# facebookresearch/SlowFast

Measured on AMD Instinct MI355X. Metric: clips/sec (fwd+bwd), SlowFast-8x8-R50 32x224^2 synthetic clips, per-GPU batch 32, higher is better.
Workload: dtype fp16; 1 GPU; SLOWFAST_8x8_R50: forward + cross_entropy loss + backward + sgd step, inputs resident in HBM, per-GPU batch 32; global_batch=32, parallelism=dp1, launch=hip-graph(fwd+bwd) + eager all-reduce/optimizer, optimizer=FlatOptimizer (fused unscale+norm+clip+update, dynamic loss scale on device)

## Files before the change

include/sfamd.h:

```cpp
#ifndef SFAMD_H
#define SFAMD_H
#include <stddef.h>
#include <stdint.h>
#ifdef __cplusplus
extern "C" {
#endif

#define SF_ABI_VERSION 32
typedef void* sf_stream_t;

typedef struct sf_conv_desc {
    int32_t N, Ci, Ti, Hi, Wi;
    int32_t Co, To, Ho, Wo;
    int32_t kT, kH, kW;
    int32_t sT, sH, sW;
    int32_t pT, pH, pW;
    int32_t dT, dH, dW;
    int32_t Cw;
    int32_t ldx, ldy;
    int32_t Cow;
} sf_conv_desc;

int sf_abi_version(void);
const char* sf_backend(void);
// ... 51 lines not shown
                     int32_t ldy, const float* scale, const float* shift, int relu_self, float* part,
                     sf_stream_t stream);
int sf_bn_bwd_finalize(float* part, int32_t nblk, int32_t C, int32_t Creal, float count, const float* gamma, const float* mean,
                       const float* rstd, float inv_loss_scale, float* dgamma, float* dbeta, int accumulate,
                       float* coef, sf_stream_t stream);
int sf_bn_bwd_apply(int64_t M, int32_t C, const void* dz, int32_t lddz, const void* zmask, int32_t ldm, const void* y,
                    int32_t ldy, const float* scale, const float* shift, int relu_self, const float* coef, void* dy,
                    int32_t lddy, void* gout, int32_t ldg, sf_stream_t stream);

int sf_pool_fwd(int32_t N, int32_t T, int32_t H, int32_t W, int32_t C, int32_t kH, int32_t kW, int32_t sH, int32_t sW,
                int32_t pH, int32_t pW, const void* y, int32_t ldy, const float* scale, const float* shift, int relu,
                void* out, int32_t ldo, void* argmax, int32_t cls, sf_stream_t stream);
int sf_pool_bwd(int32_t N, int32_t T, int32_t H, int32_t W, int32_t C, int32_t kH, int32_t kW, int32_t sH, int32_t sW,
                int32_t pH, int32_t pW, const void* pooled, int32_t ldp, const void* argmax, int relu,
                const void* dout, int32_t lddo, void* g, int32_t ldg, int32_t cls, sf_stream_t stream);

int sf_pool3d_fwd(int32_t N, int32_t T, int32_t H, int32_t W, int32_t C, int32_t kT, int32_t kH, int32_t kW, const void* x,
                  int32_t ldx, void* out, int32_t ldo, void* argmax, sf_stream_t stream);
int sf_pool3d_bwd(int32_t N, int32_t T, int32_t H, int32_t W, int32_t C, int32_t kT, int32_t kH, int32_t kW,
                  const void* argmax, const void* dout, int32_t lddo, void* dx, int32_t lddx, sf_stream_t stream);

int sf_ncthw_to_cl(const float* x, int32_t N, int32_t C, int64_t S, int32_t Cp, void* out, sf_stream_t stream);
int sf_cl_to_ncthw(const void* x, int32_t ld, int32_t N, int32_t C, int64_t S, float* out, sf_stream_t stream);


int sf_bgemm(int64_t M, int32_t N, int32_t K, const void* A, int32_t lda, const void* W, int32_t ldw, const float* bias,
             const void* resid, int32_t ldr, void* Y, int32_t ldy, int32_t nbatch, int32_t bh, int64_t sa_b, int64_t sa_h,
             int64_t sw_b, int64_t sw_h, int64_t sy_b, int64_t sy_h, int64_t sr_b, int64_t sr_h, int32_t resid_row0,
             float alpha, sf_stream_t stream);
typedef struct sf_rows32 {
// ... 222 lines not shown
```

slowfast_amd/csrc/sf_api.hip:

```cpp
#include "../../include/sfamd.h"
#include "sf_bn.h"
#include "sf_common.h"
#include "sf_igemm.h"
#include "sf_igemm2.h"
#include "sf_wgrad2.h"
#include "sf_cbwd.h"
#include "sf_pool.h"
#include "sf_dwconv.h"
#include "sf_dwsweep.h"
#include "sf_dwtemporal.h"
#include "sf_tokens.h"
#include "sf_x3d.h"
#include "sf_stem.h"
#include "sf_attn.h"
#include "sf_roi.h"
#include "sf_optim.h"
#include "sf_mixup.h"
#include "sf_erase.h"
#include "sf_pack.h"
#include "sf_sample.h"
#include "sf_color.h"
#include "sf_randaug.h"
#include "sf_hog.h"
#include "sf_pixel.h"
// ... 1122 lines not shown

extern "C" int sf_pool_bwd(int32_t N, int32_t T, int32_t H, int32_t W, int32_t C, int32_t kH, int32_t kW, int32_t sH,
                           int32_t sW, int32_t pH, int32_t pW, const void* pooled, int32_t ldp, const void* argmax,
                           int relu, const void* dout, int32_t lddo, void* g, int32_t ldg, int32_t cls,
                           sf_stream_t stream) {
    PoolParams p;
    if (fill_pool(p, N, T, H, W, C, kH, kW, sH, sW, pH, pW, nullptr, 0, nullptr, nullptr, relu)) return -1;
    REQUIRE(argmax && dout && g, "sf_pool_bwd: null pointer");
    (void)pooled; (void)ldp;
    p.cls = cls ? 1 : 0; p.fdT = make_fastdiv(T);
    p.out = (f16*)g; p.ldo = ldg; p.dout = (const f16*)dout; p.lddo = lddo;
    p.pooled = (const f16*)pooled; p.ldp = ldp; p.argmax = (uint8_t*)argmax;
    p.fdW = make_fastdiv(W); p.fdH = make_fastdiv(H);
    p.total = (int64_t)N * T * H * W * (C / 8);
    REQUIRE(p.total < (1ll << 31), "sf_pool_bwd: too many elements");
    p.fdsH = make_fastdiv(sH); p.fdsW = make_fastdiv(sW);
    if (kH <= 2 * sH && kW <= 2 * sW)
        hipLaunchKernelGGL(sf_pool_bwd4_kernel, dim3(pool_grid(p.total + (int64_t)N * (C / 8))), dim3(SF_THREADS), 0,
                           (hipStream_t)stream, p);
    else
        hipLaunchKernelGGL(sf_pool_bwd_kernel, dim3(pool_grid(p.total + (int64_t)N * (C / 8))), dim3(SF_THREADS), 0,
                           (hipStream_t)stream, p);
    return check_launch("pool_bwd");
}

extern "C" int sf_pool3d_fwd(int32_t N, int32_t T, int32_t H, int32_t W, int32_t C, int32_t kT, int32_t kH, int32_t kW,
                             const void* x, int32_t ldx, void* out, int32_t ldo, void* argmax, sf_stream_t stream) {
    REQUIRE(x && out && argmax && C > 0 && C % 8 == 0 && kT > 0 && kH > 0 && kW > 0 && kT * kH * kW <= 255,
            "sf_pool3d_fwd: bad arguments");
    Pool3dParams p;
    p.N = N; p.T = T; p.H = H; p.W = W; p.C = C; p.kT = kT; p.kH = kH; p.kW = kW;
    p.To = T / kT; p.Ho = H / kH; p.Wo = W / kW;
    REQUIRE(p.To > 0 && p.Ho > 0 && p.Wo > 0, "sf_pool3d_fwd: window larger than the input");
    p.x = (const f16*)x; p.ldx = ldx; p.out = (f16*)out; p.ldo = ldo; p.argmax = (uint8_t*)argmax;
    p.dout = nullptr; p.lddo = 0;
    p.fdG = make_fastdiv(C / 8); p.fdW = make_fastdiv(p.Wo); p.fdH = make_fastdiv(p.Ho); p.fdT = make_fastdiv(p.To);
    p.total = (int64_t)N * p.To * p.Ho * p.Wo * (C / 8);
    REQUIRE(p.total < (1ll << 31), "sf_pool3d_fwd: too many elements");
// ... 2079 lines not shown
```

slowfast_amd/csrc/sf_bn.h:

```cpp
#pragma once
#include "sf_common.h"

struct RowTile {
    int M, C;
    int rows_per_block;
    __device__ __forceinline__ bool init(int& gcol, int& r0, int& r1, int& rstep, int bx = (int)blockIdx.x) const {
        const int G = C >> 3;
        const int TG = G < SF_THREADS ? G : SF_THREADS;
        const int rpi = SF_THREADS / TG;
        const int tx = threadIdx.x % TG, ty = threadIdx.x / TG;
        gcol = blockIdx.y * SF_THREADS + tx;
        r0 = bx * rows_per_block + ty;
        r1 = (bx + 1) * rows_per_block;
        if (r1 > M) r1 = M;
        rstep = rpi;
        return ty < rpi && gcol < G;
    }
};

__device__ __forceinline__ void load8f(const float* p, float (&v)[8]) {
#pragma unroll
    for (int e = 0; e < 8; ++e) v[e] = p[e];
}

// ... 227 lines not shown
    for (int e = 0; e < 8; ++e) g[e] = (float)dz[e];
    if (bits_ptr) {
        const uint32_t b = *bits_ptr;
#pragma unroll
        for (int e = 0; e < 8; ++e) g[e] = ((b >> e) & 1u) ? g[e] : 0.f;
    } else if (zmask_ptr) {
        f16x8 z = ld16(zmask_ptr);
#pragma unroll
        for (int e = 0; e < 8; ++e) g[e] = ((float)z[e] > 0.f) ? g[e] : 0.f;
    } else if (relu_self) {
#pragma unroll
        for (int e = 0; e < 8; ++e) g[e] = ((float)yv[e] * sc[e] + sh[e] > 0.f) ? g[e] : 0.f;
    }
}

__global__ __launch_bounds__(SF_THREADS) void sf_bn_bwd_reduce_kernel(BnBwdReduceParams p) {
    __shared__ float s_red[SF_THREADS][17];
    int gcol, r0, r1, rstep;
    const bool active = p.rt.init(gcol, r0, r1, rstep);
    const int c = gcol * 8;
    float sg[8], sgy[8], sc[8], sh[8];
#pragma unroll
    for (int e = 0; e < 8; ++e) { sg[e] = 0.f; sgy[e] = 0.f; sc[e] = 1.f; sh[e] = 0.f; }
    if (active) {
        if (p.relu_self) { load8f(p.scale + c, sc); load8f(p.shift + c, sh); }
        for (int m = r0; m < r1; m += rstep) {
            f16x8 dz = ld16(p.dz + (int64_t)m * p.lddz + c);
            f16x8 yv = ld16(p.y + (int64_t)m * p.ldy + c);
            float g[8];
            const bool bitm = p.zmask && p.ldm == 0;
            masked_grad8(dz, yv, (p.zmask && !bitm) ? p.zmask + (int64_t)m * p.ldm + c : nullptr, p.relu_self, sc, sh, g,
                         bitm ? reinterpret_cast<const uint8_t*>(p.zmask) + (int64_t)m * (p.rt.C >> 3) + gcol : nullptr);
#pragma unroll
            for (int e = 0; e < 8; ++e) { sg[e] += g[e]; sgy[e] += g[e] * (float)yv[e]; }
        }
    }
    rowtile_reduce_store(p.rt, active, c, sg, sgy, p.part + (int64_t)blockIdx.x * 2 * p.rt.C, s_red);
}

struct BnBwdFinalizeParams {
    const float* part; int nblk; int row_stride; int C; int Creal;
    float count;
    const float* gamma; const float* mean; const float* rstd;
    float inv_loss_scale;
    float* dgamma; float* dbeta;
    int accumulate;
    float* coef;
};

__global__ __launch_bounds__(SF_FIN_THREADS_MAX) void sf_bn_bwd_finalize_kernel(BnBwdFinalizeParams p) {
    __shared__ double s_s[SF_FIN_SEG_MAX][SF_FIN_CH];
    __shared__ double s_q[SF_FIN_SEG_MAX][SF_FIN_CH];
// ... 25 lines not shown

struct BnBwdApplyParams {
    RowTile rt;
    const f16* dz; int lddz;
    const f16* zmask; int ldm;
    const f16* y; int ldy;
    const float* scale; const float* shift;
    int relu_self;
    const float* coef;
    f16* dy; int lddy;
    f16* gout; int ldg;
    const float* sample_add;
    FastDiv fdS;
};

__global__ __launch_bounds__(SF_THREADS) void sf_bn_bwd_apply_kernel(BnBwdApplyParams p) {
    int gcol, r0, r1, rstep;
    if (!p.rt.init(gcol, r0, r1, rstep)) return;
    const int c = gcol * 8, C = p.rt.C;
    float sc[8], sh[8], k1[8], k2[8], k3[8];
#pragma unroll
    for (int e = 0; e < 8; ++e) { sc[e] = 1.f; sh[e] = 0.f; }
    if (p.relu_self) { load8f(p.scale + c, sc); load8f(p.shift + c, sh); }
    load8f(p.coef + c, k1);
    load8f(p.coef + C + c, k2);
    load8f(p.coef + 2 * C + c, k3);
    for (int m = r0; m < r1; m += rstep) {
        f16x8 dz = ld16(p.dz + (int64_t)m * p.lddz + c);
        f16x8 yv = ld16(p.y + (int64_t)m * p.ldy + c);
        float g[8];
        const bool bitm = p.zmask && p.ldm == 0;
        masked_grad8(dz, yv, (p.zmask && !bitm) ? p.zmask + (int64_t)m * p.ldm + c : nullptr, p.relu_self, sc, sh, g,
                     bitm ? reinterpret_cast<const uint8_t*>(p.zmask) + (int64_t)m * (C >> 3) + gcol : nullptr);
        f16x8 o;
        if (p.sample_add) {
            float ad[8];
            load8f(p.sample_add + (int64_t)fd_div((uint32_t)m, p.fdS) * C + c, ad);
#pragma unroll
            for (int e = 0; e < 8; ++e) g[e] += ad[e];
        }
#pragma unroll
        for (int e = 0; e < 8; ++e) o[e] = (f16)(k1[e] * g[e] + k2[e] + k3[e] * (float)yv[e]);
        st16(p.dy + (int64_t)m * p.lddy + c, o);
        if (p.gout) {
            f16x8 go;
#pragma unroll
            for (int e = 0; e < 8; ++e) go[e] = (f16)g[e];
            st16(p.gout + (int64_t)m * p.ldg + c, go);
        }
    }
}
```

slowfast_amd/csrc/sf_pool.h:

```cpp
#pragma once
#include "sf_common.h"

struct PoolParams {
    const f16* y; int ldy;
    const float* scale; const float* shift; int relu;
    int N, T, H, W, C;
    int Ho, Wo;
    int kH, kW, sH, sW, pH, pW;
    f16* out; int ldo;
    uint8_t* argmax;
    const f16* pooled; int ldp;
    const f16* dout; int lddo;
    FastDiv fdG, fdW, fdH;
    int64_t total;
    int cls;
    FastDiv fdT;
    FastDiv fdsH, fdsW;
};

__device__ __forceinline__ int64_t pool_row(const PoolParams& p, uint32_t nt, int Hx, int Wx, int h, int w) {
    int64_t r = ((int64_t)nt * Hx + h) * Wx + w;
    if (p.cls) r += fd_div(nt, p.fdT) + 1;
    return r;
}
// ... 108 lines not shown
                const f16x8 d = ld16(p.dout + orow * p.lddo + c);
#pragma unroll
                for (int e = 0; e < 8; ++e) {
                    const uint32_t a = ((e < 4 ? pk.x : pk.y) >> (8 * (e & 3))) & 0xffu;
                    g[e] += a == me ? (float)d[e] : 0.f;
                }
            }
        }
        f16x8 o;
#pragma unroll
        for (int e = 0; e < 8; ++e) o[e] = (f16)g[e];
        st16(p.out + pool_row(p, nt, p.H, p.W, (int)h, (int)w) * p.ldo + c, o);
    }
}

__global__ __launch_bounds__(SF_THREADS) void sf_pool_bwd4_kernel(PoolParams p) {
    const int64_t ncls = p.cls ? (int64_t)p.N * (p.C >> 3) : 0;
    for (int64_t idx = (int64_t)blockIdx.x * SF_THREADS + threadIdx.x; idx < p.total + ncls;
         idx += (int64_t)gridDim.x * SF_THREADS) {
        if (idx >= p.total) {
            const int64_t j = idx - p.total;
            const int G = p.C >> 3;
            const int64_t n = j / G;
            const int c = (int)(j % G) * 8;
            st16(p.out + n * ((int64_t)p.T * p.H * p.W + 1) * p.ldo + c,
                 ld16(p.dout + n * ((int64_t)p.T * p.Ho * p.Wo + 1) * p.lddo + c));
            continue;
        }
        uint32_t q, gcol, w, h, nt;
        fd_divmod((uint32_t)idx, p.fdG, q, gcol);
        fd_divmod(q, p.fdW, q, w);
        fd_divmod(q, p.fdH, nt, h);
        const int c = gcol * 8;
        const int hh = (int)fd_div(h + (uint32_t)p.pH, p.fdsH), wh = (int)fd_div(w + (uint32_t)p.pW, p.fdsW);
        int hoc[2], woc[2], khs[2], kws[2];
        bool hv[2], wv[2];
#pragma unroll
        for (int a = 0; a < 2; ++a) {
            const int ho = hh - 1 + a, wo = wh - 1 + a;
            khs[a] = (int)h - (ho * p.sH - p.pH);
            kws[a] = (int)w - (wo * p.sW - p.pW);
            hv[a] = ho >= 0 && ho < p.Ho && khs[a] < p.kH;
            wv[a] = wo >= 0 && wo < p.Wo && kws[a] < p.kW;
            hoc[a] = ho < 0 ? 0 : (ho > p.Ho - 1 ? p.Ho - 1 : ho);
            woc[a] = wo < 0 ? 0 : (wo > p.Wo - 1 ? p.Wo - 1 : wo);
        }
        u32x2 pk[2][2];
        f16x8 d[2][2];
#pragma unroll
        for (int a = 0; a < 2; ++a)
#pragma unroll
            for (int b = 0; b < 2; ++b) {
                const int64_t orow = pool_row(p, nt, p.Ho, p.Wo, hoc[a], woc[b]);
                pk[a][b] = *reinterpret_cast<const u32x2*>(p.argmax + orow * p.C + c);
                d[a][b] = ld16(p.dout + orow * p.lddo + c);
            }
        float g[8];
#pragma unroll
        for (int e = 0; e < 8; ++e) g[e] = 0.f;
#pragma unroll
        for (int a = 0; a < 2; ++a)
#pragma unroll
            for (int b = 0; b < 2; ++b) {
                const bool on = hv[a] && wv[b];
                const uint32_t me = (uint32_t)(khs[a] * p.kW + kws[b]);
#pragma unroll
                for (int e = 0; e < 8; ++e) {
                    const uint32_t am = ((e < 4 ? pk[a][b].x : pk[a][b].y) >> (8 * (e & 3))) & 0xffu;
                    g[e] += on && am == me ? (float)d[a][b][e] : 0.f;
                }
            }
        f16x8 o;
#pragma unroll
        for (int e = 0; e < 8; ++e) o[e] = (f16)g[e];
        st16(p.out + pool_row(p, nt, p.H, p.W, (int)h, (int)w) * p.ldo + c, o);
    }
}

struct Pool3dParams {
    int N, T, H, W, C, kT, kH, kW, To, Ho, Wo;
    const f16* x; int ldx;
    f16* out; int ldo;
    uint8_t* argmax;
    const f16* dout; int lddo;
    FastDiv fdG, fdW, fdH, fdT;
    int64_t total;
};
__global__ __launch_bounds__(SF_THREADS) void sf_pool3d_fwd_kernel(Pool3dParams p) {
    for (int64_t idx = (int64_t)blockIdx.x * SF_THREADS + threadIdx.x; idx < p.total;
         idx += (int64_t)gridDim.x * SF_THREADS) {
        uint32_t q, gcol, wo, ho, to, n;
// ... 239 lines not shown
```

slowfast_amd/engine.py:

```python
import functools
import os

import torch

from . import lib as _sflib

from . import ops

_f16 = _sflib.act_dtype()
_listeners = []
FORCE_WEIGHT_PREP = False
PARAM_EPOCH = 0
PACK_RECORD = None
PACK_PLAN = os.environ.get("SF_PACK_PLAN", "1") != "0"
BN_FUSE_REDUCE = os.environ.get("SF_BN_FUSE_REDUCE", "1") != "0"
CAT_IN_PLACE = os.environ.get("SF_CAT_IN_PLACE", "1") != "0"
SEGMENTS = None


class _Segments:
    def __init__(self):
        self.cuts = []

    def cut(self, tensors):
# ... 373 lines not shown
        return geom if ops.conv_c_bwd_plan(geom) is not None else None

    def fused_c_backward(self, geom, x, dz, y, st, bits, part=None, bn_fuse=None):
        bn = self.bn
        dgamma, dbeta, accumulate = self._bn_grad_dest()
        coef = ops.bn_bwd_coef(dz, y, bn.weight, st.mean, st.rstd, dgamma, dbeta, zmask=bits, inv_loss_scale=1.0,
                               accumulate=accumulate, part=part)
        dw, zero_first = _grad_dest(self.conv.weight)
        _, wd = self.weights(geom)
        fuse = None
        if bn_fuse is not None:
            y0, st0 = bn_fuse
            fuse = (y0, st0.scale, st0.shift)
        return ops.conv_c_bwd(dz, bits, y, coef, x, wd, geom, dw, bn=fuse, out_scale=1.0, zero_first=zero_first)

    def bn_backward(self, dz, y, st, zmask=None, relu_self=False, want_g=False, part=None):
        bn = self.bn
        dgamma, dbeta, accumulate = self._bn_grad_dest()
        return ops.bn_bwd(dz, y, bn.weight, st.mean, st.rstd, dgamma, dbeta, zmask=zmask,
                          relu_affine=(st.scale, st.shift) if relu_self else None, inv_loss_scale=1.0,
                          accumulate=accumulate, want_g=want_g, sync=_sync_of(bn), part=part)

    def params(self):
        p = [self.conv.weight]
        if self.conv.bias is not None:
            p.append(self.conv.bias)
        if self.bn is not None:
            p += [self.bn.weight, self.bn.bias]
        return p

    def _fold_source(self, w):
        return w

    def fold(self):
        w = self.conv.weight.detach().float()
        b = self.conv.bias.detach().float() if self.conv.bias is not None else None
# ... 107 lines not shown
        assert k[0] == 1 and s[0] == 1 and p[0] == 0, "stem pooling is spatial-only in every reference config"
        out, arg = ops.pool_fwd(y, k[1:], s[1:], p[1:], affine=(st.scale, st.shift, True))
        if CAPTURE is not None:
            CAPTURE.append({"kind": "stem", "mod": mod, "raw": [y], "bn": [(st.scale, st.shift)], "out": out,
                            "argmax": torch.where(arg == 255, torch.zeros_like(arg), arg)})
        ctx.mod, ctx.xcl, ctx.y, ctx.st = mod, xcl, y, st
        ctx.pool = (tuple(k[1:]), tuple(s[1:]), tuple(p[1:]))
        ctx.pooled, ctx.arg = out, arg
        return out

    @staticmethod
    @delivers_grads
    def backward(ctx, dout):
        unit = ctx.mod._unit
        st = ctx.st
        g = ops.pool_bwd(ctx.y.shape, ctx.pooled, ctx.arg, as_cl(dout), *ctx.pool, relu=True)
        dy = unit.bn_backward(g, ctx.y, st)
        unit.backward(ctx.xcl, None, dy, need_dx=False)
        _notify(unit.params())
        ctx.xcl = ctx.y = ctx.pooled = ctx.arg = None
        return (None, None) + param_grads(ctx, 2)


class FuseFn(torch.autograd.Function):

    @staticmethod
    def forward(ctx, x_s, x_f, mod, *params):
        record_params(ctx, params)
        unit = mod._unit
        x_s, x_f = as_cl(x_s), as_cl(x_f)
        yf, st = unit.forward(x_f, None, mod.training)
        N, Cs, T, H, W = x_s.shape
# ... 165 lines not shown
```

slowfast_amd/lib.py:

```python
import ctypes
import os
from ctypes import POINTER, Structure, c_char_p, c_float, c_int, c_int32, c_int64, c_void_p

_HERE = os.path.dirname(os.path.abspath(__file__))
ABI_VERSION = 32
ACT_MODE = os.environ.get("SF_ACT_DTYPE", "fp16").lower()
if ACT_MODE not in ("fp16", "bf16"):
    raise ValueError(f"SF_ACT_DTYPE={ACT_MODE!r}: expected fp16 or bf16")
DEFAULT_LIBRARY = os.path.join(_HERE, "libsfamd.so" if ACT_MODE == "fp16" else "libsfamd_bf16.so")


def act_dtype():
    import torch
    return torch.float16 if ACT_MODE == "fp16" else torch.bfloat16


def act_eps():
    return 2.0 ** -11 if ACT_MODE == "fp16" else 2.0 ** -8


class ConvDesc(Structure):

    _fields_ = [(n, c_int32) for n in (
        "N", "Ci", "Ti", "Hi", "Wi", "Co", "To", "Ho", "Wo", "kT", "kH", "kW", "sT", "sH", "sW",
# ... 61 lines not shown
    "sf_bn_bwd_blocks": (c_int, [c_int64, c_int32]),
    "sf_flat_blocks": (c_int, [c_int64]),
    "sf_flat_sumsq": (c_int, [_F, c_int64, _F, _P]),
    "sf_step_control": (c_int, [_F, c_int32, _F, c_float, c_float, c_int, c_float, c_float, c_int32, _P]),
    "sf_flat_sgd": (c_int, [_F, _F, _F, _P, _P, _P, c_int32, _F, _P, _P, c_int32, c_float, c_float, c_float, c_int, _P]),
    "sf_flat_adamw": (c_int, [_F, _F, _F, _F, _P, _P, _P, c_int32, _F, _P, _P, c_int32, c_float, c_float, c_float, c_float, _P]),
    "sf_flat_sgd_tab": (c_int, [_F, _F, _F, _P, _P, _P, c_int32, _F, _F, _F, c_float, c_float, c_float, c_int, _P]),
    "sf_flat_adamw_tab": (c_int, [_F, _F, _F, _F, _P, _P, _P, c_int32, _F, _F, _F, c_float, c_float, c_float, c_float, _P]),
    "sf_flat_lars_trust": (c_int, [_F, _F, _P, _P, _P, c_int32, _P, c_int32, _F, _F, _P, _F, c_float, c_float, c_float, _P]),
    "sf_bn_bwd_reduce": (c_int, [c_int64, c_int32, _P, c_int32, _P, c_int32, _P, c_int32, _F, _F, c_int, _F, _P]),
    "sf_bn_bwd_finalize": (c_int, [_F, c_int32, c_int32, c_int32, c_float, _F, _F, _F, c_float, _F, _F, c_int, _F, _P]),
    "sf_bn_bwd_apply": (c_int, [c_int64, c_int32, _P, c_int32, _P, c_int32, _P, c_int32, _F, _F, c_int, _F, _P,
                                c_int32, _P, c_int32, _P]),
    "sf_pool_fwd": (c_int, [c_int32] * 11 + [_P, c_int32, _F, _F, c_int, _P, c_int32, _P, c_int32, _P]),
    "sf_pool_bwd": (c_int, [c_int32] * 11 + [_P, c_int32, _P, c_int, _P, c_int32, _P, c_int32, c_int32, _P]),
    "sf_pool3d_fwd": (c_int, [c_int32] * 8 + [_P, c_int32, _P, c_int32, _P, _P]),
    "sf_pool3d_bwd": (c_int, [c_int32] * 8 + [_P, _P, c_int32, _P, c_int32, _P]),
    "sf_ncthw_to_cl": (c_int, [_F, c_int32, c_int32, c_int64, c_int32, _P, _P]),
    "sf_cl_to_ncthw": (c_int, [_P, c_int32, c_int32, c_int32, c_int64, _F, _P]),
    "sf_bgemm": (c_int, [c_int64, c_int32, c_int32, _P, c_int32, _P, c_int32, _F, _P, c_int32, _P, c_int32, c_int32,
                         c_int32] + [c_int64] * 8 + [c_int32, c_float, _P]),
    "sf_bgemm_tn": (c_int, [c_int64, c_int32, c_int32, _P, c_int32, _P, c_int32, _P, c_int32, c_float, c_int32, c_int32]
                    + [c_int64] * 6 + [_P]),
    "sf_layernorm_fwd": (c_int, [c_int64, c_int32, _P, c_int32, _F, _F, c_float, _P, c_int32, _F, _F, _P]),
    "sf_gemm_rows32": (c_int, [c_int64, c_int32, c_int32, _P, c_int32, _P, c_int32, _F, _P, c_int32, _P, c_int32,
                               POINTER(Rows32), _P]),
    "sf_layernorm_fwd_rows32": (c_int, [c_int64, c_int32, _P, c_int32, _F, _F, c_float, _P, c_int32, _F, _F,
                                        POINTER(Rows32), _P]),
    "sf_layernorm_bwd_blocks": (c_int, [c_int64, c_int32]),
    "sf_layernorm_bwd": (c_int, [c_int64, c_int32, _P, c_int32, _P, c_int32, _F, _F, _F, _P, c_int32, _P, c_int32, _F, _P]),
# ... 160 lines not shown
```

slowfast_amd/ops.py:

```python
from ctypes import byref, c_int32, c_int64

import torch

from . import lib as _sflib

from .lib import ConvDesc, SfError, get_lib

_f16 = _sflib.act_dtype()


def _triple(v):
    return tuple(v) if isinstance(v, (tuple, list)) else (v, v, v)


def _stream(t):
    if t.is_cuda:
        return torch.cuda.current_stream(t.device).cuda_stream
    if get_lib().backend != "hostsim":
        raise SfError("slowfast_amd kernels need CUDA/HIP tensors (got a CPU tensor and the gfx950 library)")
    return None


def _ptr(t):
    return None if t is None else t.data_ptr()
# ... 283 lines not shown

def bn_act(y, scale=None, shift=None, relu=False, resid=None, rscale=None, rshift=None, out=None, want_mask=False):
    ldy = cl_ld(y)
    N, C, T, H, W = y.shape
    out = cl_empty(y.shape, y.device) if out is None else out
    assert tuple(out.shape) == tuple(y.shape)
    mask = torch.empty((rows(y), C // 8), dtype=torch.uint8, device=y.device) if want_mask else None
    get_lib().call("sf_bn_act", rows(y), C, y.data_ptr(), ldy, _ptr(scale), _ptr(shift), _ptr(resid),
                   cl_ld(resid) if resid is not None else 0, _ptr(rscale), _ptr(rshift), int(bool(relu)),
                   out.data_ptr(), cl_ld(out), _ptr(mask), _stream(y),
                   work=dict(bytes=2.0 * y.numel() * (2 + int(resid is not None) + (1 / 16 if want_mask else 0))))
    return (out, mask) if want_mask else out


def bn_bwd(dz, y, gamma, mean, rstd, dgamma, dbeta, zmask=None, relu_affine=None, inv_loss_scale=1.0,
           accumulate=False, want_g=False, out=None, sync=None, part=None, sample_add=None, coef_only=False):
    lib = get_lib()
    N, C, T, H, W = y.shape
    M = rows(y)
    s = _stream(y)
    fused_part = part
    if fused_part is None:
        nblk = lib.call("sf_bn_bwd_blocks", M, C)
        part = torch.empty((nblk, 2, C), dtype=torch.float32, device=y.device)
    else:
        assert part.dtype == torch.float32 and part.is_contiguous() and tuple(part.shape[1:]) == (2, C)
        nblk = part.shape[0]
    sc, sh = (relu_affine if relu_affine is not None else (None, None))
    relu_self = int(relu_affine is not None)
    bits = zmask is not None and zmask.dtype == torch.uint8
    if bits:
        assert zmask.numel() == M * (C // 8) and zmask.is_contiguous()
    mcost = 0.0 if zmask is None else (1 / 16 if bits else 1.0)
    lddz, ldy, ldm = cl_ld(dz), cl_ld(y), (0 if bits or zmask is None else cl_ld(zmask))
    if fused_part is None:
        lib.call("sf_bn_bwd_reduce", M, C, dz.data_ptr(), lddz, _ptr(zmask), ldm, y.data_ptr(), ldy, _ptr(sc), _ptr(sh),
                 relu_self, part.data_ptr(), s, work=dict(bytes=2.0 * y.numel() * (2 + mcost)))
    coef = torch.empty((3, C), dtype=torch.float32, device=y.device)
    if sync is None:
        lib.call("sf_bn_bwd_finalize", part.data_ptr(), nblk, C, gamma.numel(), float(M), gamma.data_ptr(), mean.data_ptr(),
                 rstd.data_ptr(), float(inv_loss_scale), dgamma.data_ptr(), dbeta.data_ptr(), int(accumulate),
                 coef.data_ptr(), s)
    else:
        import torch.distributed as dist
        group, gsize = sync
        tot = part.sum(0, keepdim=True)
        loc = tot.clone()
        lib.call("sf_bn_bwd_finalize", loc.data_ptr(), 1, C, gamma.numel(), float(M), gamma.data_ptr(), mean.data_ptr(),
                 rstd.data_ptr(), float(inv_loss_scale), dgamma.data_ptr(), dbeta.data_ptr(), int(accumulate),
                 coef.data_ptr(), s)
        dist.all_reduce(tot, group=group)
        scratch = torch.empty((2, gamma.numel()), dtype=torch.float32, device=y.device)
        lib.call("sf_bn_bwd_finalize", tot.data_ptr(), 1, C, gamma.numel(), float(M) * gsize, gamma.data_ptr(),
                 mean.data_ptr(), rstd.data_ptr(), float(inv_loss_scale), scratch[0].data_ptr(), scratch[1].data_ptr(), 0,
                 coef.data_ptr(), s)
    if coef_only:
        return coef
    dy = cl_empty(y.shape, y.device) if out is None else out
    if sample_add is not None:
        assert fused_part is not None and zmask is None and relu_affine is None and not want_g
        assert sample_add.dtype == torch.float32 and sample_add.is_contiguous() and tuple(sample_add.shape) == (N, C)
        lib.call("sf_bn_bwd_apply_sample", M, C, dz.data_ptr(), lddz, y.data_ptr(), ldy, coef.data_ptr(), sample_add.data_ptr(),
                 M // N, dy.data_ptr(), cl_ld(dy), s, work=dict(bytes=2.0 * y.numel() * 3))
        return dy
    g = cl_empty(y.shape, y.device) if want_g else None
    lib.call("sf_bn_bwd_apply", M, C, dz.data_ptr(), lddz, _ptr(zmask), ldm, y.data_ptr(), ldy, _ptr(sc), _ptr(sh),
             relu_self, coef.data_ptr(), dy.data_ptr(), cl_ld(dy), _ptr(g), cl_ld(g) if g is not None else 0, s,
             work=dict(bytes=2.0 * y.numel() * (3 + mcost + int(want_g))))
    return (dy, g) if want_g else dy


def bn_bwd_coef(dz, y, gamma, mean, rstd, dgamma, dbeta, zmask=None, inv_loss_scale=1.0, accumulate=False, part=None):
    return bn_bwd(dz, y, gamma, mean, rstd, dgamma, dbeta, zmask=zmask, inv_loss_scale=inv_loss_scale, accumulate=accumulate,
                  part=part, coef_only=True)


def conv_c_bwd_plan(geom, in_affine=False, mask_bits=True):
    tile_rows, ws = c_int32(0), c_int64(0)
    ok = get_lib().call("sf_conv_c_bwd_plan", byref(geom.desc(geom.Ci, geom.Co)), int(bool(in_affine)), int(bool(mask_bits)),
                        byref(tile_rows), byref(ws))
    return (tile_rows.value, ws.value) if ok == 1 else None


def conv_c_bwd(dz, bits, yc, coef, act, wd, geom, dw, bn=None, out_scale=1.0, zero_first=True, out=None):
    plan = conv_c_bwd_plan(geom)
    assert plan is not None, "conv_c_bwd: the planner rejects this geometry"
    tile_rows, ws_bytes = plan
    assert tuple(act.shape) == geom.in_shape and tuple(dz.shape) == geom.out_shape and tuple(yc.shape) == geom.out_shape
    assert dw.dtype == torch.float32 and dw.is_contiguous() and dw.numel() == geom.Cow * geom.Cw * geom.taps
# ... 50 lines not shown
```

Before: 904.2 clips/s.

## Fuse stem max-pool backward gather into BN backward reduce and apply kernels

The stem pool's backward no longer materializes the unpooled gradient tensor. The BN backward reduce and apply kernels now recompute the 2x2 argmax gather from the pooled gradient on the fly, so one full-resolution write and two reads of the stem activation gradient are avoided. The gather is done twice (once in reduce, once in apply), which adds index arithmetic and repeated small reads of argmax and dout. A test hook can switch the new path off, and the original path remains as a fallback.

```diff
diff --git a/include/sfamd.h b/include/sfamd.h
--- a/include/sfamd.h
+++ b/include/sfamd.h
@@ -6,7 +6,7 @@
 extern "C" {
 #endif
 
-#define SF_ABI_VERSION 32
+#define SF_ABI_VERSION 33
 typedef void* sf_stream_t;
 
 typedef struct sf_conv_desc {
@@ -89,6 +89,15 @@
 int sf_pool_bwd(int32_t N, int32_t T, int32_t H, int32_t W, int32_t C, int32_t kH, int32_t kW, int32_t sH, int32_t sW,
                 int32_t pH, int32_t pW, const void* pooled, int32_t ldp, const void* argmax, int relu,
                 const void* dout, int32_t lddo, void* g, int32_t ldg, int32_t cls, sf_stream_t stream);
+
+int sf_bn_bwd_pool_plan(int32_t C, int32_t kH, int32_t kW, int32_t sH, int32_t sW, int32_t cls);
+int sf_bn_bwd_reduce_pool(int32_t N, int32_t T, int32_t H, int32_t W, int32_t C, int32_t kH, int32_t kW, int32_t sH, int32_t sW,
+                          int32_t pH, int32_t pW, const void* argmax, const void* dout, int32_t lddo, const void* y, int32_t ldy,
+                          const float* scale, const float* shift, int relu_self, float* part, sf_stream_t stream);
+int sf_bn_bwd_apply_pool(int32_t N, int32_t T, int32_t H, int32_t W, int32_t C, int32_t kH, int32_t kW, int32_t sH, int32_t sW,
+                         int32_t pH, int32_t pW, const void* argmax, const void* dout, int32_t lddo, const void* y, int32_t ldy,
+                         const float* scale, const float* shift, int relu_self, const float* coef, void* dy, int32_t lddy,
+                         sf_stream_t stream);
 
 int sf_pool3d_fwd(int32_t N, int32_t T, int32_t H, int32_t W, int32_t C, int32_t kT, int32_t kH, int32_t kW, const void* x,
                   int32_t ldx, void* out, int32_t ldo, void* argmax, sf_stream_t stream);
diff --git a/slowfast_amd/csrc/sf_api.hip b/slowfast_amd/csrc/sf_api.hip
--- a/slowfast_amd/csrc/sf_api.hip
+++ b/slowfast_amd/csrc/sf_api.hip
@@ -1160,6 +1160,7 @@
     p.fdW = make_fastdiv(W); p.fdH = make_fastdiv(H);
     p.total = (int64_t)N * T * H * W * (C / 8);
     REQUIRE(p.total < (1ll << 31), "sf_pool_bwd: too many elements");
+    REQUIRE((int64_t)N * T * p.Ho * p.Wo + N < (1ll << 31), "sf_pool_bwd: too many pooled positions");
     p.fdsH = make_fastdiv(sH); p.fdsW = make_fastdiv(sW);
     if (kH <= 2 * sH && kW <= 2 * sW)
         hipLaunchKernelGGL(sf_pool_bwd4_kernel, dim3(pool_grid(p.total + (int64_t)N * (C / 8))), dim3(SF_THREADS), 0,
@@ -1168,6 +1169,70 @@
         hipLaunchKernelGGL(sf_pool_bwd_kernel, dim3(pool_grid(p.total + (int64_t)N * (C / 8))), dim3(SF_THREADS), 0,
                            (hipStream_t)stream, p);
     return check_launch("pool_bwd");
+}
+
+extern "C" int sf_bn_bwd_pool_plan(int32_t C, int32_t kH, int32_t kW, int32_t sH, int32_t sW, int32_t cls) {
+    if (test_hook("SF_STEM_POOL_FUSE", 1) == 0) return 0;
+    return C > 0 && C % 8 == 0 && kH > 0 && kW > 0 && sH > 0 && sW > 0 && kH <= 2 * sH && kW <= 2 * sW && !cls ? 1 : 0;
+}
+static int fill_pool_grad(const char* who, PoolParams& q, int32_t N, int32_t T, int32_t H, int32_t W, int32_t C, int32_t kH,
+                          int32_t kW, int32_t sH, int32_t sW, int32_t pH, int32_t pW, const void* argmax, const void* dout,
+                          int32_t lddo, int64_t& M) {
+    REQUIRE(sf_bn_bwd_pool_plan(C, kH, kW, sH, sW, 0) == 1,
+            "%s: this pool keeps sf_pool_bwd + sf_bn_bwd_reduce + sf_bn_bwd_apply (sf_bn_bwd_pool_plan == 0)", who);
+    REQUIRE(N > 0 && T > 0 && H > 0 && W > 0 && pH >= 0 && pW >= 0 && pH < kH && pW < kW && H + 2 * pH >= kH && W + 2 * pW >= kW,
+            "%s: bad pool geometry", who);
+    if (fill_pool(q, N, T, H, W, C, kH, kW, sH, sW, pH, pW, nullptr, 0, nullptr, nullptr, 1)) return -1;
+    REQUIRE(argmax && dout && lddo >= C, "%s: null pointer or short pitch", who);
+    M = (int64_t)N * T * H * W;
+    if (check_rows(who, M, C)) return -1;
+    REQUIRE((int64_t)N * T * q.Ho * q.Wo < (1ll << 31), "%s: too many pooled positions", who);
+    q.cls = 0; q.fdT = make_fastdiv(T);
+    q.dout = (const f16*)dout; q.lddo = lddo; q.argmax = (uint8_t*)argmax;
+    q.fdW = make_fastdiv(W); q.fdH = make_fastdiv(H);
+    q.fdsH = make_fastdiv(sH); q.fdsW = make_fastdiv(sW);
+    q.total = M * (C / 8);
+    return 0;
+}
+
+extern "C" int sf_bn_bwd_reduce_pool(int32_t N, int32_t T, int32_t H, int32_t W, int32_t C, int32_t kH, int32_t kW, int32_t sH,
+                                     int32_t sW, int32_t pH, int32_t pW, const void* argmax, const void* dout, int32_t lddo,
+                                     const void* y, int32_t ldy, const float* scale, const float* shift, int relu_self,
+                                     float* part, sf_stream_t stream) {
+    PoolParams q;
+    int64_t M;
+    if (fill_pool_grad("sf_bn_bwd_reduce_pool", q, N, T, H, W, C, kH, kW, sH, sW, pH, pW, argmax, dout, lddo, M)) return -1;
+    REQUIRE(y && part && ldy >= C, "sf_bn_bwd_reduce_pool: null pointer or short pitch");
+    REQUIRE(!relu_self || (scale && shift), "sf_bn_bwd_reduce_pool: relu_self needs scale/shift");
+    BnBwdReduceParams p;
+    dim3 grid;
+    p.rt = make_rowtile(M, C, kBwdBlocks, grid);
+    p.dz = nullptr; p.lddz = 0; p.zmask = nullptr; p.ldm = 0;
+    p.y = (const f16*)y; p.ldy = ldy; p.scale = scale; p.shift = shift; p.relu_self = relu_self; p.part = part;
+    if (relu_self) hipLaunchKernelGGL(sf_bn_bwd_reduce_pool_kernel<true>, grid, dim3(SF_THREADS), 0, (hipStream_t)stream, p, q);
+    else hipLaunchKernelGGL(sf_bn_bwd_reduce_pool_kernel<false>, grid, dim3(SF_THREADS), 0, (hipStream_t)stream, p, q);
+    return check_launch("bn_bwd_reduce_pool");
+}
+
+extern "C" int sf_bn_bwd_apply_pool(int32_t N, int32_t T, int32_t H, int32_t W, int32_t C, int32_t kH, int32_t kW, int32_t sH,
+                                    int32_t sW, int32_t pH, int32_t pW, const void* argmax, const void* dout, int32_t lddo,
+                                    const void* y, int32_t ldy, const float* scale, const float* shift, int relu_self,
+                                    const float* coef, void* dy, int32_t lddy, sf_stream_t stream) {
+    PoolParams q;
+    int64_t M;
+    if (fill_pool_grad("sf_bn_bwd_apply_pool", q, N, T, H, W, C, kH, kW, sH, sW, pH, pW, argmax, dout, lddo, M)) return -1;
+    REQUIRE(y && coef && dy && ldy >= C && lddy >= C, "sf_bn_bwd_apply_pool: null pointer or short pitch");
+    REQUIRE(!relu_self || (scale && shift), "sf_bn_bwd_apply_pool: relu_self needs scale/shift");
+    BnBwdApplyParams p;
+    dim3 grid;
+    p.rt = make_rowtile(M, C, 8192, grid);
+    p.dz = nullptr; p.lddz = 0; p.zmask = nullptr; p.ldm = 0;
+    p.y = (const f16*)y; p.ldy = ldy; p.scale = scale; p.shift = shift; p.relu_self = relu_self;
+    p.coef = coef; p.dy = (f16*)dy; p.lddy = lddy; p.gout = nullptr; p.ldg = 0;
+    p.sample_add = nullptr; p.fdS = make_fastdiv(1);
+    if (relu_self) hipLaunchKernelGGL(sf_bn_bwd_apply_pool_kernel<true>, grid, dim3(SF_THREADS), 0, (hipStream_t)stream, p, q);
+    else hipLaunchKernelGGL(sf_bn_bwd_apply_pool_kernel<false>, grid, dim3(SF_THREADS), 0, (hipStream_t)stream, p, q);
+    return check_launch("bn_bwd_apply_pool");
 }
 
 extern "C" int sf_pool3d_fwd(int32_t N, int32_t T, int32_t H, int32_t W, int32_t C, int32_t kT, int32_t kH, int32_t kW,
diff --git a/slowfast_amd/csrc/sf_bn.h b/slowfast_amd/csrc/sf_bn.h
--- a/slowfast_amd/csrc/sf_bn.h
+++ b/slowfast_amd/csrc/sf_bn.h
@@ -265,28 +265,44 @@
     }
 }
 
-__global__ __launch_bounds__(SF_THREADS) void sf_bn_bwd_reduce_kernel(BnBwdReduceParams p) {
-    __shared__ float s_red[SF_THREADS][17];
+struct RowGrad {
+    static constexpr bool kGatherOnly = false;
+    static constexpr int kRowsInFlight = 1;
+    static constexpr int kReluSelf = -1;
+    const f16* dz; int lddz;
+    __device__ __forceinline__ f16x8 operator()(int m, int c) const { return ld16(dz + (int64_t)m * lddz + c); }
+};
+
+template <class Src>
+__device__ __forceinline__ void bn_bwd_reduce_body(const BnBwdReduceParams& p, const Src& src, float (*s_red)[17]) {
     int gcol, r0, r1, rstep;
     const bool active = p.rt.init(gcol, r0, r1, rstep);
     const int c = gcol * 8;
     float sg[8], sgy[8], sc[8], sh[8];
 #pragma unroll
     for (int e = 0; e < 8; ++e) { sg[e] = 0.f; sgy[e] = 0.f; sc[e] = 1.f; sh[e] = 0.f; }
+    const int relu_self = Src::kReluSelf < 0 ? p.relu_self : Src::kReluSelf;
     if (active) {
-        if (p.relu_self) { load8f(p.scale + c, sc); load8f(p.shift + c, sh); }
+        if (relu_self) { load8f(p.scale + c, sc); load8f(p.shift + c, sh); }
+#pragma unroll Src::kRowsInFlight
         for (int m = r0; m < r1; m += rstep) {
-            f16x8 dz = ld16(p.dz + (int64_t)m * p.lddz + c);
             f16x8 yv = ld16(p.y + (int64_t)m * p.ldy + c);
+            f16x8 dz = src(m, c);
             float g[8];
-            const bool bitm = p.zmask && p.ldm == 0;
-            masked_grad8(dz, yv, (p.zmask && !bitm) ? p.zmask + (int64_t)m * p.ldm + c : nullptr, p.relu_self, sc, sh, g,
+            const bool zm = !Src::kGatherOnly && p.zmask;
+            const bool bitm = zm && p.ldm == 0;
+            masked_grad8(dz, yv, (zm && !bitm) ? p.zmask + (int64_t)m * p.ldm + c : nullptr, relu_self, sc, sh, g,
                          bitm ? reinterpret_cast<const uint8_t*>(p.zmask) + (int64_t)m * (p.rt.C >> 3) + gcol : nullptr);
 #pragma unroll
             for (int e = 0; e < 8; ++e) { sg[e] += g[e]; sgy[e] += g[e] * (float)yv[e]; }
         }
     }
     rowtile_reduce_store(p.rt, active, c, sg, sgy, p.part + (int64_t)blockIdx.x * 2 * p.rt.C, s_red);
+}
+
+__global__ __launch_bounds__(SF_THREADS) void sf_bn_bwd_reduce_kernel(BnBwdReduceParams p) {
+    __shared__ float s_red[SF_THREADS][17];
+    bn_bwd_reduce_body(p, RowGrad{p.dz, p.lddz}, s_red);
 }
 
 struct BnBwdFinalizeParams {
@@ -342,35 +358,50 @@
     FastDiv fdS;
 };
 
-__global__ __launch_bounds__(SF_THREADS) void sf_bn_bwd_apply_kernel(BnBwdApplyParams p) {
+__device__ __forceinline__ float bn_dy_pinned(float k1, float g, float k2, float k3, float y) {
+#if !defined(SF_HOSTSIM)
+    return __builtin_fmaf(k3, y, __builtin_fmaf(k1, g, k2));
+#else
+    return k1 * g + k2 + k3 * y;
+#endif
+}
+
+template <class Src>
+__device__ __forceinline__ void bn_bwd_apply_body(const BnBwdApplyParams& p, const Src& src) {
     int gcol, r0, r1, rstep;
     if (!p.rt.init(gcol, r0, r1, rstep)) return;
     const int c = gcol * 8, C = p.rt.C;
     float sc[8], sh[8], k1[8], k2[8], k3[8];
 #pragma unroll
     for (int e = 0; e < 8; ++e) { sc[e] = 1.f; sh[e] = 0.f; }
-    if (p.relu_self) { load8f(p.scale + c, sc); load8f(p.shift + c, sh); }
+    const int relu_self = Src::kReluSelf < 0 ? p.relu_self : Src::kReluSelf;
+    if (relu_self) { load8f(p.scale + c, sc); load8f(p.shift + c, sh); }
     load8f(p.coef + c, k1);
     load8f(p.coef + C + c, k2);
     load8f(p.coef + 2 * C + c, k3);
+#pragma unroll Src::kRowsInFlight
     for (int m = r0; m < r1; m += rstep) {
-        f16x8 dz = ld16(p.dz + (int64_t)m * p.lddz + c);
         f16x8 yv = ld16(p.y + (int64_t)m * p.ldy + c);
+        f16x8 dz = src(m, c);
         float g[8];
-        const bool bitm = p.zmask && p.ldm == 0;
-        masked_grad8(dz, yv, (p.zmask && !bitm) ? p.zmask + (int64_t)m * p.ldm + c : nullptr, p.relu_self, sc, sh, g,
+        const bool zm = !Src::kGatherOnly && p.zmask;
+        const bool bitm = zm && p.ldm == 0;
+        masked_grad8(dz, yv, (zm && !bitm) ? p.zmask + (int64_t)m * p.ldm + c : nullptr, relu_self, sc, sh, g,
                      bitm ? reinterpret_cast<const uint8_t*>(p.zmask) + (int64_t)m * (C >> 3) + gcol : nullptr);
         f16x8 o;
-        if (p.sample_add) {
+        if (!Src::kGatherOnly && p.sample_add) {
             float ad[8];
             load8f(p.sample_add + (int64_t)fd_div((uint32_t)m, p.fdS) * C + c, ad);
 #pragma unroll
             for (int e = 0; e < 8; ++e) g[e] += ad[e];
         }
 #pragma unroll
-        for (int e = 0; e < 8; ++e) o[e] = (f16)(k1[e] * g[e] + k2[e] + k3[e] * (float)yv[e]);
+        for (int e = 0; e < 8; ++e) {
+            if constexpr (Src::kGatherOnly) o[e] = (f16)bn_dy_pinned(k1[e], g[e], k2[e], k3[e], (float)yv[e]);
+            else o[e] = (f16)(k1[e] * g[e] + k2[e] + k3[e] * (float)yv[e]);
+        }
         st16(p.dy + (int64_t)m * p.lddy + c, o);
-        if (p.gout) {
+        if (!Src::kGatherOnly && p.gout) {
             f16x8 go;
 #pragma unroll
             for (int e = 0; e < 8; ++e) go[e] = (f16)g[e];
@@ -378,3 +409,7 @@
         }
     }
 }
+
+__global__ __launch_bounds__(SF_THREADS) void sf_bn_bwd_apply_kernel(BnBwdApplyParams p) {
+    bn_bwd_apply_body(p, RowGrad{p.dz, p.lddz});
+}
diff --git a/slowfast_amd/csrc/sf_pool.h b/slowfast_amd/csrc/sf_pool.h
--- a/slowfast_amd/csrc/sf_pool.h
+++ b/slowfast_amd/csrc/sf_pool.h
@@ -1,4 +1,5 @@
 #pragma once
+#include "sf_bn.h"
 #include "sf_common.h"
 
 struct PoolParams {
@@ -146,6 +147,51 @@
     }
 }
 
+__device__ __forceinline__ void pool_gather4(const PoolParams& p, uint32_t nt, uint32_t h, uint32_t w, int c, float (&g)[8]) {
+    const int hh = (int)fd_div(h + (uint32_t)p.pH, p.fdsH), wh = (int)fd_div(w + (uint32_t)p.pW, p.fdsW);
+    int hoc[2], woc[2], khs[2], kws[2];
+    bool hv[2], wv[2];
+    const int kh1 = (int)h - (hh * p.sH - p.pH), kw1 = (int)w - (wh * p.sW - p.pW);
+#pragma unroll
+    for (int a = 0; a < 2; ++a) {
+        const int ho = hh - 1 + a, wo = wh - 1 + a;
+        khs[a] = a ? kh1 : kh1 + p.sH;
+        kws[a] = a ? kw1 : kw1 + p.sW;
+        hv[a] = ho >= 0 && ho < p.Ho && khs[a] < p.kH;
+        wv[a] = wo >= 0 && wo < p.Wo && kws[a] < p.kW;
+        hoc[a] = ho < 0 ? 0 : (ho > p.Ho - 1 ? p.Ho - 1 : ho);
+        woc[a] = wo < 0 ? 0 : (wo > p.Wo - 1 ? p.Wo - 1 : wo);
+    }
+    uint32_t o00 = (nt * (uint32_t)p.Ho + (uint32_t)hoc[0]) * (uint32_t)p.Wo + (uint32_t)woc[0];
+    if (p.cls) o00 += fd_div(nt, p.fdT) + 1;
+    const uint8_t* ap = p.argmax + (int64_t)o00 * p.C + c;
+    const f16* dp = p.dout + (int64_t)o00 * p.lddo + c;
+    const int ah = hoc[1] != hoc[0] ? p.Wo * p.C : 0, aw = woc[1] != woc[0] ? p.C : 0;
+    const int dh = hoc[1] != hoc[0] ? p.Wo * p.lddo : 0, dw = woc[1] != woc[0] ? p.lddo : 0;
+    u32x2 pk[2][2];
+    f16x8 d[2][2];
+#pragma unroll
+    for (int a = 0; a < 2; ++a)
+#pragma unroll
+        for (int b = 0; b < 2; ++b) {
+            pk[a][b] = *reinterpret_cast<const u32x2*>(ap + (a ? ah : 0) + (b ? aw : 0));
+            d[a][b] = ld16(dp + (a ? dh : 0) + (b ? dw : 0));
+        }
+#pragma unroll
+    for (int e = 0; e < 8; ++e) g[e] = 0.f;
+#pragma unroll
+    for (int a = 0; a < 2; ++a)
+#pragma unroll
+        for (int b = 0; b < 2; ++b) {
+            const uint32_t me = hv[a] && wv[b] ? (uint32_t)(khs[a] * p.kW + kws[b]) : 0x100u;
+#pragma unroll
+            for (int e = 0; e < 8; ++e) {
+                const uint32_t am = ((e < 4 ? pk[a][b].x : pk[a][b].y) >> (8 * (e & 3))) & 0xffu;
+                g[e] += am == me ? (float)d[a][b][e] : 0.f;
+            }
+        }
+}
+
 __global__ __launch_bounds__(SF_THREADS) void sf_pool_bwd4_kernel(PoolParams p) {
     const int64_t ncls = p.cls ? (int64_t)p.N * (p.C >> 3) : 0;
     for (int64_t idx = (int64_t)blockIdx.x * SF_THREADS + threadIdx.x; idx < p.total + ncls;
@@ -164,49 +210,45 @@
         fd_divmod(q, p.fdW, q, w);
         fd_divmod(q, p.fdH, nt, h);
         const int c = gcol * 8;
-        const int hh = (int)fd_div(h + (uint32_t)p.pH, p.fdsH), wh = (int)fd_div(w + (uint32_t)p.pW, p.fdsW);
-        int hoc[2], woc[2], khs[2], kws[2];
-        bool hv[2], wv[2];
-#pragma unroll
-        for (int a = 0; a < 2; ++a) {
-            const int ho = hh - 1 + a, wo = wh - 1 + a;
-            khs[a] = (int)h - (ho * p.sH - p.pH);
-            kws[a] = (int)w - (wo * p.sW - p.pW);
-            hv[a] = ho >= 0 && ho < p.Ho && khs[a] < p.kH;
-            wv[a] = wo >= 0 && wo < p.Wo && kws[a] < p.kW;
-            hoc[a] = ho < 0 ? 0 : (ho > p.Ho - 1 ? p.Ho - 1 : ho);
-            woc[a] = wo < 0 ? 0 : (wo > p.Wo - 1 ? p.Wo - 1 : wo);
-        }
-        u32x2 pk[2][2];
-        f16x8 d[2][2];
-#pragma unroll
-        for (int a = 0; a < 2; ++a)
-#pragma unroll
-            for (int b = 0; b < 2; ++b) {
-                const int64_t orow = pool_row(p, nt, p.Ho, p.Wo, hoc[a], woc[b]);
-                pk[a][b] = *reinterpret_cast<const u32x2*>(p.argmax + orow * p.C + c);
-                d[a][b] = ld16(p.dout + orow * p.lddo + c);
-            }
         float g[8];
-#pragma unroll
-        for (int e = 0; e < 8; ++e) g[e] = 0.f;
-#pragma unroll
-        for (int a = 0; a < 2; ++a)
-#pragma unroll
-            for (int b = 0; b < 2; ++b) {
-                const bool on = hv[a] && wv[b];
-                const uint32_t me = (uint32_t)(khs[a] * p.kW + kws[b]);
-#pragma unroll
-                for (int e = 0; e < 8; ++e) {
-                    const uint32_t am = ((e < 4 ? pk[a][b].x : pk[a][b].y) >> (8 * (e & 3))) & 0xffu;
-                    g[e] += on && am == me ? (float)d[a][b][e] : 0.f;
-                }
-            }
+        pool_gather4(p, nt, h, w, c, g);
         f16x8 o;
 #pragma unroll
         for (int e = 0; e < 8; ++e) o[e] = (f16)g[e];
         st16(p.out + pool_row(p, nt, p.H, p.W, (int)h, (int)w) * p.ldo + c, o);
     }
+}
+
+template <bool RELU, int ROWS>
+struct PoolGrad {
+    static constexpr bool kGatherOnly = true;
+    static constexpr int kReluSelf = RELU ? 1 : 0;
+    static constexpr int kRowsInFlight = ROWS;
+    const PoolParams& q;
+    __device__ __forceinline__ f16x8 operator()(int m, int c) const {
+        uint32_t r, w, h, nt;
+        fd_divmod((uint32_t)m, q.fdW, r, w);
+        fd_divmod(r, q.fdH, nt, h);
+        float g[8];
+        pool_gather4(q, nt, h, w, c, g);
+        f16x8 o;
+#pragma unroll
+        for (int e = 0; e < 8; ++e) o[e] = (f16)g[e];
+        return o;
+    }
+};
+
+#define SF_POOL_REDUCE_ROWS 2
+#define SF_POOL_APPLY_ROWS 2
+template <bool RELU>
+__global__ __launch_bounds__(SF_THREADS) void sf_bn_bwd_reduce_pool_kernel(BnBwdReduceParams p, PoolParams q) {
+    __shared__ float s_red[SF_THREADS][17];
+    bn_bwd_reduce_body(p, PoolGrad<RELU, SF_POOL_REDUCE_ROWS>{q}, s_red);
+}
+
+template <bool RELU>
+__global__ __launch_bounds__(SF_THREADS) void sf_bn_bwd_apply_pool_kernel(BnBwdApplyParams p, PoolParams q) {
+    bn_bwd_apply_body(p, PoolGrad<RELU, SF_POOL_APPLY_ROWS>{q});
 }
 
 struct Pool3dParams {
diff --git a/slowfast_amd/engine.py b/slowfast_amd/engine.py
--- a/slowfast_amd/engine.py
+++ b/slowfast_amd/engine.py
@@ -411,12 +411,12 @@
             fuse = (y0, st0.scale, st0.shift)
         return ops.conv_c_bwd(dz, bits, y, coef, x, wd, geom, dw, bn=fuse, out_scale=1.0, zero_first=zero_first)
 
-    def bn_backward(self, dz, y, st, zmask=None, relu_self=False, want_g=False, part=None):
+    def bn_backward(self, dz, y, st, zmask=None, relu_self=False, want_g=False, part=None, pool=None):
         bn = self.bn
         dgamma, dbeta, accumulate = self._bn_grad_dest()
         return ops.bn_bwd(dz, y, bn.weight, st.mean, st.rstd, dgamma, dbeta, zmask=zmask,
                           relu_affine=(st.scale, st.shift) if relu_self else None, inv_loss_scale=1.0,
-                          accumulate=accumulate, want_g=want_g, sync=_sync_of(bn), part=part)
+                          accumulate=accumulate, want_g=want_g, sync=_sync_of(bn), part=part, pool=pool)
 
     def params(self):
         p = [self.conv.weight]
@@ -554,8 +554,11 @@
     def backward(ctx, dout):
         unit = ctx.mod._unit
         st = ctx.st
-        g = ops.pool_bwd(ctx.y.shape, ctx.pooled, ctx.arg, as_cl(dout), *ctx.pool, relu=True)
-        dy = unit.bn_backward(g, ctx.y, st)
+        if ops.bn_bwd_pool_plan(ctx.y.shape[1], ctx.pool[0], ctx.pool[1]):
+            dy = unit.bn_backward(as_cl(dout), ctx.y, st, pool=(ctx.arg,) + ctx.pool)
+        else:
+            g = ops.pool_bwd(ctx.y.shape, ctx.pooled, ctx.arg, as_cl(dout), *ctx.pool, relu=True)
+            dy = unit.bn_backward(g, ctx.y, st)
         unit.backward(ctx.xcl, None, dy, need_dx=False)
         _notify(unit.params())
         ctx.xcl = ctx.y = ctx.pooled = ctx.arg = None
diff --git a/slowfast_amd/lib.py b/slowfast_amd/lib.py
--- a/slowfast_amd/lib.py
+++ b/slowfast_amd/lib.py
@@ -3,7 +3,7 @@
 from ctypes import POINTER, Structure, c_char_p, c_float, c_int, c_int32, c_int64, c_void_p
 
 _HERE = os.path.dirname(os.path.abspath(__file__))
-ABI_VERSION = 32
+ABI_VERSION = 33
 ACT_MODE = os.environ.get("SF_ACT_DTYPE", "fp16").lower()
 if ACT_MODE not in ("fp16", "bf16"):
     raise ValueError(f"SF_ACT_DTYPE={ACT_MODE!r}: expected fp16 or bf16")
@@ -99,6 +99,9 @@
                                 c_int32, _P, c_int32, _P]),
     "sf_pool_fwd": (c_int, [c_int32] * 11 + [_P, c_int32, _F, _F, c_int, _P, c_int32, _P, c_int32, _P]),
     "sf_pool_bwd": (c_int, [c_int32] * 11 + [_P, c_int32, _P, c_int, _P, c_int32, _P, c_int32, c_int32, _P]),
+    "sf_bn_bwd_pool_plan": (c_int, [c_int32] * 6),
+    "sf_bn_bwd_reduce_pool": (c_int, [c_int32] * 11 + [_P, _P, c_int32, _P, c_int32, _F, _F, c_int, _F, _P]),
+    "sf_bn_bwd_apply_pool": (c_int, [c_int32] * 11 + [_P, _P, c_int32, _P, c_int32, _F, _F, c_int, _F, _P, c_int32, _P]),
     "sf_pool3d_fwd": (c_int, [c_int32] * 8 + [_P, c_int32, _P, c_int32, _P, _P]),
     "sf_pool3d_bwd": (c_int, [c_int32] * 8 + [_P, _P, c_int32, _P, c_int32, _P]),
     "sf_ncthw_to_cl": (c_int, [_F, c_int32, c_int32, c_int64, c_int32, _P, _P]),
diff --git a/slowfast_amd/ops.py b/slowfast_amd/ops.py
--- a/slowfast_amd/ops.py
+++ b/slowfast_amd/ops.py
@@ -321,7 +321,7 @@
 
 
 def bn_bwd(dz, y, gamma, mean, rstd, dgamma, dbeta, zmask=None, relu_affine=None, inv_loss_scale=1.0,
-           accumulate=False, want_g=False, out=None, sync=None, part=None, sample_add=None, coef_only=False):
+           accumulate=False, want_g=False, out=None, sync=None, part=None, sample_add=None, coef_only=False, pool=None):
     lib = get_lib()
     N, C, T, H, W = y.shape
     M = rows(y)
@@ -335,12 +335,22 @@
         nblk = part.shape[0]
     sc, sh = (relu_affine if relu_affine is not None else (None, None))
     relu_self = int(relu_affine is not None)
+    if pool is not None:
+        assert zmask is None and fused_part is None and sample_add is None and not want_g
+        argmax, kernel, stride, padding = pool
+        pargs, (Ho, Wo) = _pool_args(y, kernel, stride, padding)
+        assert tuple(dz.shape) == (N, C, T, Ho, Wo) and argmax.dtype == torch.uint8 and argmax.is_contiguous()
+        assert argmax.numel() == dz.numel()
+        pargs += (argmax.data_ptr(), dz.data_ptr(), cl_ld(dz), y.data_ptr(), cl_ld(y), _ptr(sc), _ptr(sh), relu_self)
+        gcost = 1.5 * dz.numel()
     bits = zmask is not None and zmask.dtype == torch.uint8
     if bits:
         assert zmask.numel() == M * (C // 8) and zmask.is_contiguous()
     mcost = 0.0 if zmask is None else (1 / 16 if bits else 1.0)
     lddz, ldy, ldm = cl_ld(dz), cl_ld(y), (0 if bits or zmask is None else cl_ld(zmask))
-    if fused_part is None:
+    if pool is not None:
+        lib.call("sf_bn_bwd_reduce_pool", *pargs, part.data_ptr(), s, work=dict(bytes=2.0 * (y.numel() + gcost)))
+    elif fused_part is None:
         lib.call("sf_bn_bwd_reduce", M, C, dz.data_ptr(), lddz, _ptr(zmask), ldm, y.data_ptr(), ldy, _ptr(sc), _ptr(sh),
                  relu_self, part.data_ptr(), s, work=dict(bytes=2.0 * y.numel() * (2 + mcost)))
     coef = torch.empty((3, C), dtype=torch.float32, device=y.device)
@@ -364,6 +374,10 @@
     if coef_only:
         return coef
     dy = cl_empty(y.shape, y.device) if out is None else out
+    if pool is not None:
+        lib.call("sf_bn_bwd_apply_pool", *pargs, coef.data_ptr(), dy.data_ptr(), cl_ld(dy), s,
+                 work=dict(bytes=2.0 * (2 * y.numel() + gcost)))
+        return dy
     if sample_add is not None:
         assert fused_part is not None and zmask is None and relu_affine is None and not want_g
         assert sample_add.dtype == torch.float32 and sample_add.is_contiguous() and tuple(sample_add.shape) == (N, C)
@@ -380,6 +394,11 @@
 def bn_bwd_coef(dz, y, gamma, mean, rstd, dgamma, dbeta, zmask=None, inv_loss_scale=1.0, accumulate=False, part=None):
     return bn_bwd(dz, y, gamma, mean, rstd, dgamma, dbeta, zmask=zmask, inv_loss_scale=inv_loss_scale, accumulate=accumulate,
                   part=part, coef_only=True)
+
+
+def bn_bwd_pool_plan(C, kernel, stride, cls=False):
+    (kH, kW), (sH, sW) = kernel, stride
+    return get_lib().call("sf_bn_bwd_pool_plan", C, kH, kW, sH, sW, int(bool(cls))) == 1
 
 
 def conv_c_bwd_plan(geom, in_affine=False, mask_bits=True):
```

Result: no change. 901.5 clips/s (-0.3%).
